# DerekRowell/AudioSDR

Hardware: AMD Instinct MI355X
Metric: Msamples/s through full SSB demod chain, batched 128-sample blocks (higher is better)
Workload: dtype f32

## Files before the change

### audiosdr_amd/csrc/asdr_kernels.hip

```cpp
#include <hip/hip_runtime.h>
#include <stdint.h>
#include <stddef.h>
#include <string.h>
#include <stdlib.h>
#include <type_traits>

#include "asdr_device.h"
#include "asdr_tables.h"
#include "../../include/asdr.h"

#ifndef ASDR_STRIDE
#define ASDR_STRIDE 388
#endif
#ifndef ASDR_ALS_STRIDE
#define ASDR_ALS_STRIDE 392
#endif
#ifndef ASDR_PRE_STRIDE
#define ASDR_PRE_STRIDE 260
#endif
#ifndef ASDR_MW
#define ASDR_MW 1
#endif
#ifndef ASDR_MW_MIN_WAVES
#define ASDR_MW_MIN_WAVES 64
#endif
#ifndef ASDR_MW_SHARE
#define ASDR_MW_SHARE 7
#endif
#ifndef ASDR_MW_PRIO
#define ASDR_MW_PRIO 2
#endif
#ifndef ASDR_MW_FIR_RING
#define ASDR_MW_FIR_RING 1
#endif
#ifndef ASDR_C16
#define ASDR_C16 0
#endif
#ifndef ASDR_C16_MIN_WAVES
#define ASDR_C16_MIN_WAVES 64
#endif
#ifndef ASDR_STATE_POLICY
#define ASDR_STATE_POLICY 1
#endif
#ifndef ASDR_NT_LOADS
#define ASDR_NT_LOADS 2
#endif
#ifndef ASDR_PIPE_PK_MASK
#define ASDR_PIPE_PK_MASK 8
#endif
#ifndef ASDR_PIPE_CHUNK
#define ASDR_PIPE_CHUNK 8
#endif
#ifndef ASDR_WAVES_PER_EU
#define ASDR_WAVES_PER_EU 3
#endif
#ifndef ASDR_ALS_WAVES_PER_EU
#define ASDR_ALS_WAVES_PER_EU 3
#endif
#ifndef ASDR_ALS_K_WAVES_PER_EU
#define ASDR_ALS_K_WAVES_PER_EU 3
#endif
#ifndef ASDR_POST_BOUNDS
#define ASDR_POST_BOUNDS ASDR_WAVES_PER_EU
#endif
#ifndef ASDR_PLL_LANES
#define ASDR_PLL_LANES 64
#endif
#ifndef ASDR_ABLATE
#define ASDR_ABLATE 0
#endif
#ifndef ASDR_STREAM_R1_CARRY
#define ASDR_STREAM_R1_CARRY 0
#endif
#ifndef ASDR_PIPE_BANK_SELECT
#define ASDR_PIPE_BANK_SELECT 0
#endif

#define W0 0
#define W1 128
#define PH 256
#define XP 0
#define ASDR_COMPACT_ROWS(stride) ((stride) < 500)
#define SCR0 387
#define NB_B 2
#define NB_MSKB 0
#define NB_CB 68
#define AGC_GV 128
#define AGC_TAB 256
#define ALS_OUT W0

#define PI_D 3.1415926535897932384626433832795

typedef float v4f __attribute__((ext_vector_type(4)));

#define ABL_NB 1
#define ABL_IF 2
#define ABL_SAM 4
#define ABL_MIX 8
#define ABL_HIL 16
#define ABL_ENV 32
#define ABL_AF 64
#define ABL_AGC 128
#define ABL_ALS 256
#define ABL_ON(x) (!(ASDR_ABLATE & (x)))

__constant__ float c_bq_pool[ASDR_N_BQ_TABLES][ASDR_BQ_COEFS];
__constant__ float c_hilbert[ASDR_HILBERT_TAPS];
__constant__ float c_sine[ASDR_SINE_TABLE_LEN];
__constant__ float c_mask_val[8];

extern "C" int asdr_kernels_upload_tables(void) {
  if (hipMemcpyToSymbol(HIP_SYMBOL(c_bq_pool), asdr_bq_pool, sizeof(asdr_bq_pool)) != hipSuccess) return -1;
  if (hipMemcpyToSymbol(HIP_SYMBOL(c_hilbert), asdr_hilbert_taps, sizeof(asdr_hilbert_taps)) != hipSuccess) return -1;
  if (hipMemcpyToSymbol(HIP_SYMBOL(c_sine), asdr_sine_table, sizeof(asdr_sine_table)) != hipSuccess) return -1;
  {
    const float val[8] = {0.0f, 1.0f, (float)0.933, (float)0.750, (float)0.500, (float)0.250, (float)0.067, 1.0f};
    if (hipMemcpyToSymbol(HIP_SYMBOL(c_mask_val), val, sizeof val) != hipSuccess) return -1;
  }
  return 0;
}

#ifdef ASDR_FENCE
#define SCHED_FENCE() __builtin_amdgcn_sched_barrier(0)
#else
#define SCHED_FENCE() do { } while (0)
#endif
#include "asdr_fir.h"
__device__ __forceinline__ double div_by_const(double x, double c, double r) {
  const double q0 = x * r;
  const double rem = __builtin_fma(-q0, c, x);
  return __builtin_fma(rem, r, q0);
// ... 136 lines not shown
  auto step = [&](auto edge_tag, const int c) {
    constexpr bool EDGE = decltype(edge_tag)::value;
    const int cn = c - st;
    float x[C], p[C], y[C];
#if ASDR_PIPE_BANK_SELECT
#pragma unroll
    for (int j = 0; j < C; ++j) x[j] = __int_as_float(__builtin_amdgcn_update_dpp(__float_as_int(xn[j]), __float_as_int(yo[j]), 0x114, 0xF, 0xE, false));
#elif ASDR_PIPE_CHUNK != 8
#pragma unroll
    for (int j = 0; j < C; ++j) { const float d = dpp_row_shr1(yo[j]); x[j] = s0 ? xn[j] : d; }
#else
    asm("s_mov_b64 vcc, %[m]\n\ts_nop 1\n\t"
        "v_cndmask_b32_dpp %[x0], %[y0], %[n0], vcc row_shr:1 row_mask:0xf bank_mask:0xf bound_ctrl:1\n\t"
        "v_cndmask_b32_dpp %[x1], %[y1], %[n1], vcc row_shr:1 row_mask:0xf bank_mask:0xf bound_ctrl:1\n\t"
        "v_cndmask_b32_dpp %[x2], %[y2], %[n2], vcc row_shr:1 row_mask:0xf bank_mask:0xf bound_ctrl:1\n\t"
        "v_cndmask_b32_dpp %[x3], %[y3], %[n3], vcc row_shr:1 row_mask:0xf bank_mask:0xf bound_ctrl:1\n\t"
        "v_cndmask_b32_dpp %[x4], %[y4], %[n4], vcc row_shr:1 row_mask:0xf bank_mask:0xf bound_ctrl:1\n\t"
        "v_cndmask_b32_dpp %[x5], %[y5], %[n5], vcc row_shr:1 row_mask:0xf bank_mask:0xf bound_ctrl:1\n\t"
        "v_cndmask_b32_dpp %[x6], %[y6], %[n6], vcc row_shr:1 row_mask:0xf bank_mask:0xf bound_ctrl:1\n\t"
        "v_cndmask_b32_dpp %[x7], %[y7], %[n7], vcc row_shr:1 row_mask:0xf bank_mask:0xf bound_ctrl:1"
        : [x0] "=&v"(x[0]), [x1] "=&v"(x[1]), [x2] "=&v"(x[2]), [x3] "=&v"(x[3]), [x4] "=&v"(x[4]), [x5] "=&v"(x[5]), [x6] "=&v"(x[6]), [x7] "=&v"(x[7])
        : [y0] "v"(yo[0]), [y1] "v"(yo[1]), [y2] "v"(yo[2]), [y3] "v"(yo[3]), [y4] "v"(yo[4]), [y5] "v"(yo[5]), [y6] "v"(yo[6]), [y7] "v"(yo[7]),
          [n0] "v"(xn[0]), [n1] "v"(xn[1]), [n2] "v"(xn[2]), [n3] "v"(xn[3]), [n4] "v"(xn[4]), [n5] "v"(xn[5]), [n6] "v"(xn[6]), [n7] "v"(xn[7]),
          [m] "s"(s0m)
        : "vcc");
#endif
    {
      const int nc = (c + 1 < ASDR_N / C) ? c + 1 : ASDR_N / C - 1;
#pragma unroll
      for (int q = 0; q < C / 4; ++q) { const float4 t = reinterpret_cast<const float4 *>(row)[nc * (C / 4) + q]; xn[4 * q] = t.x; xn[4 * q + 1] = t.y; xn[4 * q + 2] = t.z; xn[4 * q + 3] = t.w; }
    }
#if ASDR_PIPE_CHUNK == 8
    if constexpr (PK) {
    {
      const v2f B0 = (v2f){b0, b0}, B1 = (v2f){b1, b1}, B2 = (v2f){b2, b2};
      v2f P[6];
      P[0] = (v2f){x2, x[2]}; P[1] = (v2f){x1, x[3]};
#pragma unroll
      for (int k = 0; k < 4; ++k) P[2 + k] = (v2f){x[k], x[k + 4]};
#pragma unroll
      for (int k = 0; k < 4; ++k) {
        v2f t = B0 * P[2 + k]; t += B1 * P[1 + k]; t += B2 * P[k];
        p[k] = t.x; p[k + 4] = t.y;
      }
    }
    } else
#endif
    {
#pragma unroll
    for (int j = 0; j < C; ++j) {
      const float xm1 = (j >= 1) ? x[j - 1] : x1, xm2 = (j >= 2) ? x[j - 2] : ((j == 1) ? x1 : x2);
      float t = b0 * x[j]; t += b1 * xm1; t += b2 * xm2;
      p[j] = t;
    }
    }
#pragma unroll
    for (int j = 0; j < C; ++j) {
      const float ym1 = (j >= 1) ? y[j - 1] : y1, ym2 = (j >= 2) ? y[j - 2] : ((j == 1) ? y1 : y2);
      float t = p[j] + a1 * ym1; t += a2 * ym2;
      y[j] = t;
    }
    const bool act = !EDGE || ((cn >= 0) && (cn < ASDR_N / C));
    if (act) { x1 = x[C - 1]; x2 = x[C - 2]; y1 = y[C - 1]; y2 = y[C - 2]; }
#pragma unroll
    for (int j = 0; j < C; ++j) yo[j] = y[j];
    if (on && act && st == 3) {
#pragma unroll
      for (int q = 0; q < C / 4; ++q) reinterpret_cast<float4 *>(row)[cn * (C / 4) + q] = make_float4(y[4 * q], y[4 * q + 1], y[4 * q + 2], y[4 * q + 3]);
    }
  };
#if ASDR_PIPE_CHUNK != 8
#pragma unroll 1
  for (int c = 0; c < NSTEP; ++c) step(std::true_type{}, c);
#else
#pragma unroll 1
  for (int c = 0; c < 3; ++c) step(std::true_type{}, c);
#pragma unroll 1
  for (int c = 3; c < 15; c += 2) { step(std::false_type{}, c); step(std::false_type{}, c + 1); }
  step(std::false_type{}, 15);
#pragma unroll 1
  for (int c = 16; c < NSTEP; ++c) step(std::true_type{}, c);
#endif
  sv[0] = x1; sv[1] = x2; sv[2] = y1; sv[3] = y2;
}

__device__ __forceinline__ void load16(const float *p, float *v) {
  const float4 *q = reinterpret_cast<const float4 *>(p);
#pragma unroll
  for (int r = 0; r < 4; ++r) { float4 t = q[r]; v[4 * r] = t.x; v[4 * r + 1] = t.y; v[4 * r + 2] = t.z; v[4 * r + 3] = t.w; }
}
__device__ __forceinline__ void load8(const float *p, float *v) {
  const float4 *q = reinterpret_cast<const float4 *>(p);
  const float4 a = q[0], b = q[1];
  v[0] = a.x; v[1] = a.y; v[2] = a.z; v[3] = a.w; v[4] = b.x; v[5] = b.y; v[6] = b.z; v[7] = b.w;
}
__device__ __forceinline__ void load4(const float *p, float *v) {
  const float4 a = *reinterpret_cast<const float4 *>(p);
  v[0] = a.x; v[1] = a.y; v[2] = a.z; v[3] = a.w;
}
__device__ __forceinline__ void store4(float *p, const float *v) { *reinterpret_cast<float4 *>(p) = make_float4(v[0], v[1], v[2], v[3]); }
__device__ __forceinline__ void store4_nt(float *p, const float *v) {
  typedef float f4v __attribute__((ext_vector_type(4)));
  const f4v tv = {v[0], v[1], v[2], v[3]};
  __builtin_nontemporal_store(tv, reinterpret_cast<f4v *>(p));
}
__device__ __forceinline__ int4 load_int4_nt(const int4 *p) {
  typedef int i4v __attribute__((ext_vector_type(4)));
  const i4v t = __builtin_nontemporal_load(reinterpret_cast<const i4v *>(p));
  return make_int4(t[0], t[1], t[2], t[3]);
}
__device__ __forceinline__ void load4_nt(const float *p, float *v) {
  typedef float f4v __attribute__((ext_vector_type(4)));
  const f4v t = __builtin_nontemporal_load(reinterpret_cast<const f4v *>(p));
  v[0] = t[0]; v[1] = t[1]; v[2] = t[2]; v[3] = t[3];
}
__device__ __forceinline__ void store_int4_nt(int4 *p, int4 v) {
  typedef int i4v __attribute__((ext_vector_type(4)));
  const i4v tv = {v.x, v.y, v.z, v.w};
  __builtin_nontemporal_store(tv, reinterpret_cast<i4v *>(p));
}
template <bool PLAIN> __device__ __forceinline__ void store4_state(float *p, const float *v) { if constexpr (PLAIN) store4(p, v); else store4_nt(p, v); }
template <bool PLAIN> __device__ __forceinline__ void store_int4_state(int4 *p, int4 v) { if constexpr (PLAIN) *p = v; else store_int4_nt(p, v); }
__device__ __forceinline__ void store4e(float *p, const float *v) { *reinterpret_cast<float4 *>(p) = make_float4(v[0], v[2], v[4], v[6]); }
__device__ __forceinline__ void store8(float *p, const float *v) {
  float4 *q = reinterpret_cast<float4 *>(p);
  q[0] = make_float4(v[0], v[1], v[2], v[3]); q[1] = make_float4(v[4], v[5], v[6], v[7]);
}

__device__ __forceinline__ double div_i16_by_32767(double x) {
  return __builtin_fma(x, 0x1.0002000400080p-15, x * 0x1.0002000400080p-75);
}
__device__ __forceinline__ void scale8(const int16_t *s, double g, float *out, bool unit = false) {
  if (unit) {
#pragma unroll
    for (int j = 0; j < 8; ++j) { const float x = (float)s[j]; out[j] = __builtin_fmaf(x, 0x1.0002p-15f, x * 0x1.0002p-45f); }
    return;
  }
#pragma unroll
  for (int j = 0; j < 8; ++j) {
    out[j] = (float)(div_i16_by_32767((double)s[j]) * g);
    if ((j & 1) == 1) SCHED_FENCE();
  }
}
#define ASDR_MASK_MAGIC 0x14c4005000006ull
__device__ __forceinline__ float mask_decode_byte(float tabv, uint32_t group4, uint32_t word, int k) {
  const uint32_t sh = (k == 0) ? (word << 2) : (word >> (8 * k - 2));
  const uint32_t addr = (sh & 0x1Cu) | group4;
  return __int_as_float(__builtin_amdgcn_ds_bpermute((int)addr, __float_as_int(tabv)));
}
__device__ __forceinline__ uint32_t mask_encode(float v) {
  const uint32_t idx = (__float_as_uint(v) >> 21) & 0x1Fu;
  return (uint32_t)(ASDR_MASK_MAGIC >> ((idx * 3u - 36u) & 63u)) & 7u;
}
__device__ __forceinline__ uint32_t mask_encode4(float4 mv) {
  const uint32_t c0 = mask_encode(mv.x), c1 = mask_encode(mv.y), c2 = mask_encode(mv.z), c3 = mask_encode(mv.w);
  return c0 | (c1 << 8) | (c2 << 16) | (c3 << 24);
}

#define ALS_TAP(q, wh) ((((q) & 1) ? (wh) : 0) + ((q) >> 1))
template <bool CHECKED, int WH>
__device__ __forceinline__ float als_dot(const float *w, const float *x, int top, int M) {
  float y = 0.0f;
  int q = 0;
#pragma unroll 2
  for (; q + 4 <= M; q += 4) {
    const float2 we = *reinterpret_cast<const float2 *>(w + (q >> 1)), wo = *reinterpret_cast<const float2 *>(w + WH + (q >> 1));
// ... 337 lines not shown
        for (int j = 0; j < 4; ++j) XI[j] = L[XB + i0 + 4 * j];
        epoch(std::false_type{}, std::integral_constant<int, 0>{}, ep0, E, F, XI);
        epoch(std::false_type{}, std::integral_constant<int, 1>{}, ep0 + 1, E, F, XI);
        epoch(std::false_type{}, std::integral_constant<int, 2>{}, ep0 + 2, E, F, XI);
        epoch(std::false_type{}, std::integral_constant<int, 3>{}, ep0 + 3, E, F, XI);
      }
#pragma unroll
      for (int g = 0; g < 7; ++g) L[AW + WH * h + 4 * g + tq] = wr[g];
      WAVE_SYNC();
    } else
    if (__any(als_en && adaptive)) {
#pragma unroll 1
      for (int ep = -1; ep < 32; ++ep) {
        const int base = (ep < 0) ? 0 : 4 * ep + 1;
        const int cntn = (ep < 0) ? 1 : ((ep == 31) ? 3 : 4);
        const int n = base + (s8 & 3);
        const bool mine = als_en && adaptive && (s8 < cntn);
        if (als_safe) {
          const int i = 128 + n, h = s8 >> 2;
          float y = 0.0f;
          if (als_m_default) y = als_dot_split_const<ALS_M_DEFAULT>(L + AW + WH * h, L + XB + (i - D - h), h);
          else if (als_m_uniform) y = als_dot_split_uniform(L + AW + WH * h, L + XB + (i - D - h), M_u, h);
          else if (als_en && adaptive) y = als_dot_split(L + AW + WH * h, L + XB + (i - D - h), M, h);
          if (mine) {
            const float e = L[XB + i] - y;
            L[OUT + n] = notch ? e : y;
            if ((n & 3) == 0) L[SCR] = e;
          }
        } else if (mine) {
          if constexpr (!COMPACT) {
            const int i = 128 + n;
            const float y = als_dot<true, WH>(L + AW, L + XB, i - D, M);
            const float e = L[XB + i] - y;
            L[OUT + n] = notch ? e : y;
            if ((n & 3) == 0) L[SCR] = e;
          }
        }
        WAVE_SYNC();
        const int nu = (ep < 0) ? 0 : 4 * ep + 4;
        if (als_en && adaptive && nu < ASDR_N) {
          const float e = L[SCR];
          const int iu = 128 + nu;
          if (als_m_default) {
            als_tap_update_const<ALS_M_DEFAULT>(L + XB + iu - D - s8, L + AW + ALS_TAP(s8, WH), e, lam, s8);
          } else if (als_m_uniform && als_safe) {
            const float *xq = L + XB + iu - D - s8;
            float *wq = L + AW + ALS_TAP(s8, WH);
            const int nk = (M_u - s8 + 7) >> 3, nk_max = (M_u + 7) >> 3;
#pragma unroll 1
            for (int k0 = 0; k0 < nk_max; k0 += 8) {
              float xv[8], wv[8];
#pragma unroll
              for (int j = 0; j < 8; ++j) { xv[j] = xq[-8 * (k0 + j)]; wv[j] = wq[4 * (k0 + j)]; }
#pragma unroll
              for (int j = 0; j < 8; ++j) { const float gq = e * xv[j]; const float dq = lam * gq; const float wn = wv[j] + dq; wv[j] = (k0 + j < nk) ? wn : wv[j]; }
#pragma unroll
              for (int j = 0; j < 8; ++j) wq[4 * (k0 + j)] = wv[j];
            }
          } else if (als_safe) {
#pragma unroll 2
            for (int q = s8; q < M; q += 8) { const float gq = e * L[XB + iu - D - q]; const float dq = lam * gq; L[AW + ALS_TAP(q, WH)] += dq; }
          } else {
            if constexpr (!COMPACT) {
              for (int q = s8; q < M; q += 8) { const float gq = e * (((iu - D - q) >= 0 && (iu - D - q) < 256) ? L[XB + (iu - D - q)] : 0.0f); const float dq = lam * gq; L[AW + ALS_TAP(q, WH)] += dq; }
            }
          }
        }
        WAVE_SYNC();
      }
    }
}
template <int STRIDE, bool HAS_ALS, bool HAS_SAM, bool UNIFORM, int WAVES, int ROLE = 0, bool ONEBLK_ = false, int FIR_HELPERS = 1, bool UPAR = false>
__device__ __forceinline__ void asdr_update_body(const UpdateArgs &a, float *lds_wg) {
  constexpr bool C16 = (STRIDE == 320);
  constexpr bool PRE_ROLE = (ROLE == 4 || ROLE == 8), POST_ROLE = (ROLE == 5 || ROLE == 9 || ROLE == 10), LOOPED_ROLE = (ROLE == 7 || ROLE == 8 || ROLE == 9 || ROLE == 10);
  constexpr bool DO1 = (ROLE == 0 || ROLE == 1 || PRE_ROLE || ROLE == 6 || ROLE == 7), DO2 = (ROLE == 0 || ROLE == 2 || POST_ROLE || ROLE == 6 || ROLE == 7),
                 DO3 = (ROLE == 0 || ROLE == 3 || POST_ROLE || ROLE == 6 || ROLE == 7);
  constexpr bool TO_ALS = (ROLE == 6 || ROLE == 7 || ROLE == 10);
  constexpr bool ONEBLK = ONEBLK_ || (ROLE >= 4 && !LOOPED_ROLE);
  constexpr bool ALS_FULL_OPT = ASDR_COMPACT_ROWS(STRIDE) && ONEBLK;
  constexpr bool STREAM = (ROLE >= 1 && ROLE <= 3);
  constexpr bool PIPE_PK = ((ASDR_PIPE_PK_MASK & 1) && HAS_ALS) || ((ASDR_PIPE_PK_MASK & 2) && !HAS_ALS && !HAS_SAM && ROLE == 0) ||
                           ((ASDR_PIPE_PK_MASK & 4) && (HAS_SAM || ROLE > 3)) || ((ASDR_PIPE_PK_MASK & 8) && STREAM);
  if (ROLE == 0 && a.run_if != nullptr && *a.run_if == 0u) return;
  constexpr bool MW = (WAVES > 1) && !HAS_SAM && (ROLE == 0);
  constexpr int MW_SHARE = MW ? ASDR_MW_SHARE : 0;
  const int wave = (WAVES > 1) ? (int)(threadIdx.x >> 6) : 0;
  constexpr bool ORDERED = (ROLE == 0) && !HAS_ALS && !HAS_SAM && UNIFORM && ONEBLK_ && (STRIDE == ASDR_STRIDE);
  constexpr bool ST_PLAIN = ORDERED && (ASDR_STATE_POLICY >= 1), LD_PLAIN = ORDERED && (ASDR_STATE_POLICY >= 2);
  const int wg_l = (ORDERED && a.wg_reverse != 0u) ? (int)(gridDim.x - 1u - blockIdx.x) : (int)blockIdx.x;
  const int mw_rel = MW ? (int)(((uint32_t)wave - blockIdx.x) & (uint32_t)(WAVES - 1)) : 0;
  float *const mwx = lds_wg + WAVES * 8 * STRIDE;
  int *const mw_flags = reinterpret_cast<int *>(lds_wg + WAVES * 8 * STRIDE + 8 * WAVES * 16 + 260) + 4;
  constexpr int MWX = 16;
  auto mw_channel = [&](int q) -> int { const int sidx = wg_l * (8 * WAVES) + q; return (sidx < a.n_sched) ? a.direct_ch0 + sidx : a.n_channels; };
  const int wave_g = STREAM ? wg_l % a.stream_waves : wg_l * WAVES + wave;
  float *const lds = lds_wg + wave * 8 * STRIDE;
  const int lane = threadIdx.x & 63, c8 = lane >> 3, s8_ = lane & 7;
  float *const sine = HAS_SAM ? lds_wg + WAVES * 8 * STRIDE : nullptr;
  if (HAS_SAM) for (int i = lane; i < ASDR_SINE_TABLE_LEN; i += 64) sine[i] = c_sine[i];

  int4 slot = make_int4(a.n_channels, 0, 0, 0);
  const bool mw_pad = MW && (wave_g * 8 >= a.n_sched);
  if (UNIFORM && a.direct_ch0 >= 0) slot = make_int4(mw_pad ? a.n_channels : a.direct_ch0 + wave_g * 8 + c8, (int)a.direct_mode, (int)a.direct_flags, (int)((a.direct_lo & 0xFFu) | (wave_g == 0 ? a.lo_writer_bit : 0u)));
  else if (WAVES == 1 || wave_g * 8 < a.n_sched) slot = *reinterpret_cast<const int4 *>(a.sched + wave_g * 8 + c8);
  else { const ChanParams *pd = a.params + a.n_channels; slot.y = (int)pd->mode; slot.z = (int)pd->flags; }
  const int ch_ = slot.x;
  const bool valid = (UNIFORM && !mw_pad) || (ch_ < a.n_channels);
  const int loff_ = c8 * STRIDE;
#define P (*Pp)
  const ChainConsts K = a.k;
  auto pv = [](float x) -> float { if constexpr (UPAR) asm volatile("" : "+v"(x)); return x; };

  const uint32_t mode = UNIFORM ? (uint32_t)__builtin_amdgcn_readfirstlane(slot.y) : (uint32_t)slot.y;
  const uint32_t pflags = UNIFORM ? (uint32_t)__builtin_amdgcn_readfirstlane(slot.z) : (uint32_t)slot.z;
  const uint32_t lo_slot = UNIFORM ? (uint32_t)__builtin_amdgcn_readfirstlane(slot.w) : 0u;
  const bool is_ssb = DO2 && ((mode == ASDR_USBmode) || (mode == ASDR_LSBmode) || (mode == ASDR_CW_USBmode) ||
                              (mode == ASDR_CW_LSBmode) || (mode == ASDR_WSPRmode));
  const bool is_am = !C16 && (mode == ASDR_AMmode), is_sam = (HAS_SAM || ROLE >= 4) && (mode == ASDR_SAMmode);
  const bool sub_q = (mode == ASDR_USBmode) || (mode == ASDR_CW_USBmode) || (mode == ASDR_WSPRmode);
  const bool nb_en = DO1 && (pflags & ASDR_F_NB_EN), af_en = DO3 && (pflags & ASDR_F_AF_EN), agc_en = DO3 && (pflags & ASDR_F_AGC_EN);
  const bool als_en = HAS_ALS && (pflags & ASDR_F_ALS_EN);
  const bool muted = pflags & ASDR_F_MUTED;
  const float two_pi = K.two_pi_f;
  WAVE_SYNC();
  uint32_t seen_in = 0u, seen_free = 0u, seen_lo = 0u, sig_pending = 0u;
  float carry_phase = 0.0f, carry_fsh = 0.0f;
  uint32_t carry_hs = 0u;
  int4 pf_in[4] = {make_int4(0, 0, 0, 0), make_int4(0, 0, 0, 0), make_int4(0, 0, 0, 0), make_int4(0, 0, 0, 0)};
  constexpr bool R2_ONE_TRIP = (ROLE == 2) && (FIR_HELPERS == 3);
  v4f r2n_key = (v4f){0.f, 0.f, 0.f, 0.f}, r2n_c4[4], r2n_s4[4], r2n_vi[4], r2n_vq[4];
  bool r2_pref = false;
  uint32_t r2_look_in = 0u, r2_look_lo = 0u;
  float4 r1_if_s4 = make_float4(0.f, 0.f, 0.f, 0.f);
  float r1_if_cf[5] = {0.f, 0.f, 0.f, 0.f, 0.f}, r1_gain_i = 0.f, r1_gain_q = 0.f;
  uint32_t *const my_prog = STREAM ? a.stream_prog + (ROLE - 1) * a.stream_waves + wave_g : nullptr;

  constexpr bool UNIT_OK = (ONEBLK && ROLE == 0) || ROLE == 1;
  static_assert(!C16 || (ONEBLK && UNIFORM && !HAS_ALS && !HAS_SAM && WAVES == 1 && ROLE == 0), "the 16-waves-per-CU form is the plain uniform one-block kernel");
#pragma unroll 1
  for (int blk = 0; blk < (ONEBLK ? 1 : a.n_blocks); ++blk) {
    int s8 = s8_; asm volatile("" : "+v"(s8));
    int loff = loff_; asm volatile("" : "+v"(loff));
    int ch = ch_; asm volatile("" : "+v"(ch));
    int lane_i = lane; asm volatile("" : "+v"(lane_i));
#ifdef ASDR_TIMELINE
    if (STREAM && a.taps != nullptr && wave_g == 0 && lane == 0) (reinterpret_cast<unsigned long long *>(a.taps) + 64 * (3 + ROLE) + 32 * (blk & 1))[16] = clock64();
#endif
    if (STREAM) {
      uint32_t *prog = a.stream_prog, *err = a.stream_err;
      const uint32_t b1 = (uint32_t)blk + 1u, freed = (blk >= ASDR_STREAM_DEPTH) ? (uint32_t)(blk - ASDR_STREAM_DEPTH + 1) : 0u;
      const bool need_in = (ROLE != 1) && seen_in < b1, need_free = (ROLE != 3) && seen_free < freed;
      if ((need_in || need_free) && sig_pending) { stream_signal(my_prog, sig_pending, lane); sig_pending = 0u; }
      if (need_in) { seen_in = stream_wait(prog + (ROLE - 2) * a.stream_waves + wave_g, b1, err, a.stream_spin_limit); if (seen_in == ASDR_STREAM_FAIL) break; }
      if (need_free) { seen_free = stream_wait(prog + ROLE * a.stream_waves + wave_g, freed, err, a.stream_spin_limit); if (seen_free == ASDR_STREAM_FAIL) break; }
    }
    const ChanParams *Pp = UPAR ? &a.uni : row_ptr(a.params, (uint32_t)ch * (uint32_t)sizeof(ChanParams));
    ChanSmall *S = row_ptr(a.small, (uint32_t)ch * (uint32_t)sizeof(ChanSmall));
    float *L = lds + loff;
    int *Li = reinterpret_cast<int *>(L);
    constexpr bool PLB = (ASDR_PIPE_BANK_SELECT != 0);
#define pl_st (PLB ? ((lane_i & 15) >> 2) : (s8 & 3))
#define pl_iq (PLB ? (lane_i & 1) : (s8 >> 2))
#define pl_c (PLB ? (2 * (lane_i >> 4) + ((lane_i >> 1) & 1)) : (lane_i >> 3))
#define pa_c (PLB ? (2 * (lane_i >> 4) + (lane_i & 1)) : (lane_i >> 3))
#define pa_real (PLB ? ((lane_i & 3) < 2) : ((lane_i & 7) < 4))
// ... 1062 lines not shown
        }
        S->am_carrier = lvl; carrier_now = lvl; carrier_fresh = true;
        if (ROLE == 2) {
          float *xc = a.xch_c + (size_t)ch * ASDR_STREAM_DEPTH + (size_t)(blk % ASDR_STREAM_DEPTH);
          asm volatile("global_store_dword %0, %1, off sc1\n\ts_nop 0" :: "v"(xc), "v"(lvl) : "memory");
        }
      }
    }
    if (is_sam && pll_locked) {
#pragma unroll 1
      for (int h = 0; h < 2; ++h) {
        float vi[8], vq[8];
        load8(L + W0 + kA + 64 * h, vi); load8(L + W1 + kA + 64 * h, vq);
        TAP8(ASDR_TAP_MIX_I, h, vi); TAP8(ASDR_TAP_MIX_Q, h, vq);
        store8(L + W0 + kA + 64 * h, vq);
      }
    }
    if ((ROLE == 0 || ROLE == 6 || ROLE == 7) && !is_ssb && !is_am && mode != ASDR_SAMmode) {
      float z[16];
      DEFINE_ALL_PATHS(z, 16);
      if (a.audio_prev != nullptr) {
        const float *ap = row_ptr(a.audio_prev, (uint32_t)ch * 512u + 4u * (uint32_t)kF);
#pragma unroll
        for (int m = 0; m < 4; ++m) load4(ap + 32 * m, z + 4 * m);
      }
#pragma unroll
      for (int m = 0; m < 4; ++m) store4(L + W0 + kF + 32 * m, z + 4 * m);
    }
    WAVE_SYNC();
    TL(10);
    TAP_ROW(ASDR_TAP_DEMOD, W0);
    if (ROLE == 2 || ROLE == 3) {
      float *xb = a.xch_b + ((size_t)ch * ASDR_STREAM_DEPTH + (size_t)(blk % ASDR_STREAM_DEPTH)) * ASDR_N + kF;
      if (ROLE == 2) {
        v4f v[4];
#pragma unroll
        for (int m = 0; m < 4; ++m) v[m] = *reinterpret_cast<const v4f *>(L + W0 + kF + 32 * m);
        xch_store4x4(xb, v[0], v[1], v[2], v[3]);
        sig_pending = (uint32_t)blk + 1u;
        continue;
      } else {
        v4f v[4];
        if (is_am) {
          const float *xc = a.xch_c + (size_t)ch * ASDR_STREAM_DEPTH + (size_t)(blk % ASDR_STREAM_DEPTH);
          asm volatile("global_load_dword %4, %6, off sc1\n\t"
                       "global_load_dwordx4 %0, %5, off sc1\n\tglobal_load_dwordx4 %1, %5, off offset:128 sc1\n\t"
                       "global_load_dwordx4 %2, %5, off offset:256 sc1\n\tglobal_load_dwordx4 %3, %5, off offset:384 sc1\n\t"
                       "s_waitcnt vmcnt(0)"
                       : "=&v"(v[0]), "=&v"(v[1]), "=&v"(v[2]), "=&v"(v[3]), "=&v"(carrier_now) : "v"(xb), "v"(xc) : "memory");
          carrier_fresh = true;
        } else
        xch_load4x4(xb, v[0], v[1], v[2], v[3]);
        if (sig_pending) { if (lane == 0) __hip_atomic_store(my_prog, sig_pending, __ATOMIC_RELAXED, __HIP_MEMORY_SCOPE_AGENT); sig_pending = 0u; }
#pragma unroll
        for (int m = 0; m < 4; ++m) *reinterpret_cast<v4f *>(L + W0 + kF + 32 * m) = v[m];
        WAVE_SYNC();
      }
    }

    float4 agc_t4[5];
#pragma unroll
    for (int r = 0; r < 5; ++r) agc_t4[r] = make_float4(0.f, 0.f, 0.f, 0.f);
    float agc_al_a = 0.f, agc_be_a = 0.f, agc_al_r = 0.f, agc_be_r = 0.f, agc_sg = 0.f;
    uint32_t agc_hang = 0u;
    if (ABL_ON(ABL_AGC) && agc_en) {
      agc_al_a = P.agc_alpha_att; agc_be_a = P.agc_beta_att; agc_al_r = P.agc_alpha_rel; agc_be_r = P.agc_beta_rel;
      agc_sg = P.agc_static_gain; agc_hang = P.agc_hang_count;
      const float *gtab = a.agc_tab + (size_t)agc_tab_idx * ASDR_AGC_TAB_ROW;
      if constexpr (!C16) {
#pragma unroll
      for (int r = 0; r < 5; ++r) { const int q = s8 + 8 * r; if (q < 33) agc_t4[r] = reinterpret_cast<const float4 *>(gtab)[q]; }
      }
    }
    if constexpr ((MW_SHARE & 1) != 0) {
      if (ABL_ON(ABL_AF) && af_en) {
        TL(21);
        __syncthreads();
        TL(22);
        if (mw_audio_duty) {
          if (ASDR_MW_PRIO) __builtin_amdgcn_s_setprio(ASDR_MW_PRIO);
          const int st = pl_st;
          float sv[4];
          sv[0] = af_s4.x; sv[1] = af_s4.y; sv[2] = af_s4.z; sv[3] = af_s4.w;
          biquad_pipe<PIPE_PK>(lds_wg + (16 * (mw_rel - 1) + mw_casc) * STRIDE + W0, true, st, af_cf, sv);
          *reinterpret_cast<float4 *>(&mw_af_S->af_state[4 * st]) = make_float4(sv[0], sv[1], sv[2], sv[3]);
          if (ASDR_MW_PRIO) __builtin_amdgcn_s_setprio(0);
        }
        TL(23);
        __syncthreads();
        TL(24);
      }
    } else
    if (ABL_ON(ABL_AF) && __any(af_en)) {
      const int st = pl_st;
      const bool on = af_en_pa && pa_real;
      float sv[4];
      sv[0] = af_s4.x; sv[1] = af_s4.y; sv[2] = af_s4.z; sv[3] = af_s4.w;
      ChanSmall *const Saf = Spa;
      biquad_pipe<PIPE_PK>(Lpa + W0, on, st, af_cf, sv);
      if (on) *reinterpret_cast<float4 *>(&Saf->af_state[4 * st]) = make_float4(sv[0], sv[1], sv[2], sv[3]);
      WAVE_SYNC();
    }
    TL(11);
    TAP_ROW(ASDR_TAP_AUDIO_FILT, W0);

    if (ABL_ON(ABL_AGC) && __any(agc_en)) {
      const float *tab = C16 ? a.agc_tab + (size_t)agc_tab_idx * ASDR_AGC_TAB_ROW : L + AGC_TAB;
      const float gain_in = agc_gain_in;
      float av16[16];
      DEFINE_ALL_PATHS(av16, 16);
      float blockmax = 0.0f;
      if (agc_en) {
#pragma unroll
        for (int h = 0; h < 2; ++h) {
          float au[8];
          load8(L + W0 + kA + 64 * h, au);
#pragma unroll
          for (int j = 0; j < 8; ++j) { const float ax = fabsf(au[j]); av16[8 * h + j] = (ax > 1.0f) ? 1.0f : ax; }
          float mx = av16[8 * h];
#pragma unroll
          for (int u = 1; u < 8; ++u) mx = fmaxf(mx, av16[8 * h + u]);
          blockmax = (h == 0) ? mx : fmaxf(blockmax, mx);
        }
        blockmax = fmaxf(blockmax, __int_as_float(__builtin_amdgcn_update_dpp(0, __float_as_int(blockmax), 0xB1, 0xF, 0xF, true)));
        blockmax = fmaxf(blockmax, __int_as_float(__builtin_amdgcn_update_dpp(0, __float_as_int(blockmax), 0x4E, 0xF, 0xF, true)));
        blockmax = fmaxf(blockmax, __int_as_float(__builtin_amdgcn_update_dpp(0, __float_as_int(blockmax), 0x141, 0xF, 0xF, true)));
      }
      const float am_level = (float)(2.0 * (double)(carrier_fresh ? carrier_now : agc_carrier0));
      const float am_clamped = (am_level > 1.0f) ? 1.0f : am_level;
      const bool agc_quiet = __all(!(agc_en && lead) || (agc_hc0 >= 128u && agc_hang >= 8u && !((is_am ? am_clamped : blockmax) > agc_old0)));
      if (agc_en && !agc_quiet) {
        if constexpr (!C16) {
#pragma unroll
        for (int r = 0; r < 5; ++r) { const int q = s8 + 8 * r; if (q < 33) *reinterpret_cast<float4 *>(L + AGC_TAB + 4 * q) = agc_t4[r]; }
        }
        store8(L + AGC_GV + kA, av16); store8(L + AGC_GV + kA + 64, av16 + 8);
      }
      if (!agc_quiet) WAVE_SYNC();
      TL(12);
      if (agc_quiet) {
        if (agc_en && lead) {
          S->agc_hang_counter = agc_hc0 - 128u;
          status = (status & ~ASDR_S_AGC_ACTIVE) | (((double)gain_in < 0.99) ? ASDR_S_AGC_ACTIVE : 0u);
        }
      }
      {
      float agc_old_end = 0.0f; uint32_t agc_hc_end = 0u;
      auto agc_chain = [&](auto own_tag, float *Lc, ChanSmall *Sc, float old0, uint32_t hc0, float g_in, float al_a, float be_a, float al_r, float be_r, uint32_t hang,
                           bool am, float am_lvl) -> float {
        float old_abs = old0;
        uint32_t hc = hc0;
        float gv = -1.0f;
        if (am) {
#pragma unroll 1
          for (int i = 0; i < ASDR_N; i += 4) *reinterpret_cast<float4 *>(Lc + AGC_GV + i) = make_float4(am_lvl, am_lvl, am_lvl, am_lvl);
        }
        float x_[8];
        load8(Lc + AGC_GV, x_);
#pragma unroll 1
        for (int i2 = 0; i2 < ASDR_N; i2 += 16) {
          float xn_[8];
#pragma unroll
        for (int half = 0; half < 2; ++half) {
          const int i = i2 + 8 * half;
          float *x = half ? xn_ : x_, *xn = half ? x_ : xn_;
          float gvv[8];
          load8(Lc + AGC_GV + ((i + 8 < ASDR_N) ? i + 8 : i), xn);
          float mx = x[0];
#pragma unroll
          for (int u = 1; u < 8; ++u) mx = fmaxf(mx, x[u]);
          const bool no_release = __all(hc >= 8u && hang >= 8u);
          if (no_release && __all(!(mx > old_abs))) {
            hc -= 8u;
#pragma unroll
            for (int u = 0; u < 8; ++u) gvv[u] = gv;
          } else if (no_release) {
            uint32_t hcb = hc;
#pragma unroll
            for (int u = 0; u < 8; ++u) {
              const float av = x[u];
              const bool att = av > old_abs;
              if (MW || __any(att)) {
// ... 925 lines not shown
```

Before: 87790.

## Add one-sample-skew biquad cascade pipeline with inline-asm DPP handover for audio filter

Adds a new biquad cascade implementation in which each of four stage lanes is skewed by one sample and receives its input from the previous stage through a DPP row_shr:1 cndmask, written as hand-scheduled inline assembly over 8-sample chunks. It is enabled by default for the non-ALS, non-SAM role-0 path via a new mask macro and replaces the previous biquad_pipe there. The intent is to shorten the per-sample dependency chain and drop the per-step edge masking of the old skewed pipeline. In exchange it adds fragile inline asm that clobbers vcc, hand-managed write offsets, and a static_assert that rules out combining it with the packed or bank-select variants.

```diff
diff --git a/audiosdr_amd/csrc/asdr_kernels.hip b/audiosdr_amd/csrc/asdr_kernels.hip
--- a/audiosdr_amd/csrc/asdr_kernels.hip
+++ b/audiosdr_amd/csrc/asdr_kernels.hip
@@ -47,6 +47,9 @@
 #endif
 #ifndef ASDR_PIPE_PK_MASK
 #define ASDR_PIPE_PK_MASK 8
+#endif
+#ifndef ASDR_PIPE_SKEW1_MASK
+#define ASDR_PIPE_SKEW1_MASK 2
 #endif
 #ifndef ASDR_PIPE_CHUNK
 #define ASDR_PIPE_CHUNK 8
@@ -349,6 +352,94 @@
   for (int c = 16; c < NSTEP; ++c) step(std::true_type{}, c);
 #endif
   sv[0] = x1; sv[1] = x2; sv[2] = y1; sv[3] = y2;
+}
+
+__device__ __forceinline__ void load8(const float *p, float *v);
+#define ASDR_BQ_SLOT(YJ, NJ, XA, XB, YA, YB) \
+  "v_mul_f32 %[" YJ "], %[b1], %[" XA "]\n\t" \
+  "v_mul_f32 %[t1], %[b2], %[" XB "]\n\t" \
+  "v_mul_f32 %[t2], %[a1], %[" YA "]\n\t" \
+  "v_mul_f32 %[t3], %[a2], %[" YB "]\n\t" \
+  "v_cndmask_b32_dpp %[" XB "], %[" YA "], %[" NJ "], vcc row_shr:1 row_mask:0xf bank_mask:0xf bound_ctrl:1\n\t" \
+  "v_mul_f32 %[t0], %[b0], %[" XB "]\n\t" \
+  "v_add_f32 %[t0], %[t0], %[" YJ "]\n\t" \
+  "v_add_f32 %[t0], %[t0], %[t1]\n\t" \
+  "v_add_f32 %[t0], %[t0], %[t2]\n\t" \
+  "v_add_f32 %[" YJ "], %[t0], %[t3]\n\t"
+__device__ __forceinline__ void biquad_pipe_skew1(float *row, bool on, int st, const float *cf, float *sv) {
+  const float b0 = cf[0], b1 = cf[1], b2 = cf[2], a1 = cf[3], a2 = cf[4];
+  float x1 = sv[0], x2 = sv[1], y1 = sv[2], y2 = sv[3];
+  float xn[8], yp[8];
+  load8(row, xn);
+  const bool s0 = (st == 0), wr = on && (st == 3);
+  const unsigned long long s0m = __ballot(s0);
+  auto slot = [&](auto edge_tag, const int t, const float xin) -> float {
+    constexpr bool EDGE = decltype(edge_tag)::value;
+    const float d = dpp_row_shr1(y1);
+    const float x = s0 ? xin : d;
+    float acc = b0 * x; acc += b1 * x1; acc += b2 * x2; acc += a1 * y1; acc += a2 * y2;
+    if constexpr (EDGE) {
+      const int n = t - st;
+      const bool act = (n >= 0 && n < ASDR_N);
+      asm volatile("" : "+v"(acc));
+      x2 = act ? x1 : x2; x1 = act ? x : x1; y2 = act ? y1 : y2; y1 = act ? acc : y1;
+    } else { x2 = x1; x1 = x; y2 = y1; y1 = acc; }
+    return acc;
+  };
+  {
+    float nx[8];
+    load8(row + 8, nx);
+#pragma unroll
+    for (int j = 0; j < 3; ++j) yp[j] = slot(std::true_type{}, j, xn[j]);
+#pragma unroll
+    for (int j = 3; j < 8; ++j) yp[j] = slot(std::false_type{}, j, xn[j]);
+#pragma unroll
+    for (int j = 0; j < 8; ++j) xn[j] = nx[j];
+  }
+  auto step = [&](auto pf_tag, const int c) {
+    constexpr bool PF = decltype(pf_tag)::value;
+    float nx[8], y[8], t0, t1, t2, t3;
+    if constexpr (PF) load8(row + 8 * (c + 1), nx);
+    asm("s_mov_b64 vcc, %[m]\n\t"
+        ASDR_BQ_SLOT("y0", "n0", "xa", "xb", "p1", "p2")
+        ASDR_BQ_SLOT("y1", "n1", "xb", "xa", "y0", "p1")
+        ASDR_BQ_SLOT("y2", "n2", "xa", "xb", "y1", "y0")
+        ASDR_BQ_SLOT("y3", "n3", "xb", "xa", "y2", "y1")
+        ASDR_BQ_SLOT("y4", "n4", "xa", "xb", "y3", "y2")
+        ASDR_BQ_SLOT("y5", "n5", "xb", "xa", "y4", "y3")
+        ASDR_BQ_SLOT("y6", "n6", "xa", "xb", "y5", "y4")
+        ASDR_BQ_SLOT("y7", "n7", "xb", "xa", "y6", "y5")
+        : [y0] "=&v"(y[0]), [y1] "=&v"(y[1]), [y2] "=&v"(y[2]), [y3] "=&v"(y[3]), [y4] "=&v"(y[4]), [y5] "=&v"(y[5]), [y6] "=&v"(y[6]), [y7] "=&v"(y[7]),
+          [t0] "=&v"(t0), [t1] "=&v"(t1), [t2] "=&v"(t2), [t3] "=&v"(t3), [xa] "+v"(x1), [xb] "+v"(x2)
+        : [n0] "v"(xn[0]), [n1] "v"(xn[1]), [n2] "v"(xn[2]), [n3] "v"(xn[3]), [n4] "v"(xn[4]), [n5] "v"(xn[5]), [n6] "v"(xn[6]), [n7] "v"(xn[7]),
+          [b0] "v"(b0), [b1] "v"(b1), [b2] "v"(b2), [a1] "v"(a1), [a2] "v"(a2), [p1] "v"(y1), [p2] "v"(y2), [m] "s"(s0m)
+        : "vcc");
+    y1 = y[7]; y2 = y[6];
+    if (wr) {
+      float4 *const o = reinterpret_cast<float4 *>(row + 8 * (c - 1));
+      o[0] = make_float4(yp[3], yp[4], yp[5], yp[6]); o[1] = make_float4(yp[7], y[0], y[1], y[2]);
+    }
+#pragma unroll
+    for (int j = 0; j < 8; ++j) { yp[j] = y[j]; if constexpr (PF) xn[j] = nx[j]; }
+  };
+#pragma unroll 1
+  for (int c = 1; c < 15; c += 2) { step(std::true_type{}, c); step(std::true_type{}, c + 1); }
+  step(std::false_type{}, 15);
+  {
+    float y[3];
+#pragma unroll
+    for (int j = 0; j < 3; ++j) y[j] = slot(std::true_type{}, ASDR_N + j, 0.0f);
+    if (wr) {
+      float4 *const o = reinterpret_cast<float4 *>(row + ASDR_N - 8);
+      o[0] = make_float4(yp[3], yp[4], yp[5], yp[6]); o[1] = make_float4(yp[7], y[0], y[1], y[2]);
+    }
+  }
+  sv[0] = x1; sv[1] = x2; sv[2] = y1; sv[3] = y2;
+}
+#undef ASDR_BQ_SLOT
+template <bool PK, bool SKEW1>
+__device__ __forceinline__ void biquad_run(float *row, bool on, int st, const float *cf, float *sv) {
+  if constexpr (SKEW1) biquad_pipe_skew1(row, on, st, cf, sv); else biquad_pipe<PK>(row, on, st, cf, sv);
 }
 
 __device__ __forceinline__ void load16(const float *p, float *v) {
@@ -852,6 +943,9 @@
   constexpr bool STREAM = (ROLE >= 1 && ROLE <= 3);
   constexpr bool PIPE_PK = ((ASDR_PIPE_PK_MASK & 1) && HAS_ALS) || ((ASDR_PIPE_PK_MASK & 2) && !HAS_ALS && !HAS_SAM && ROLE == 0) ||
                            ((ASDR_PIPE_PK_MASK & 4) && (HAS_SAM || ROLE > 3)) || ((ASDR_PIPE_PK_MASK & 8) && STREAM);
+  constexpr bool PIPE_SKEW1 = !STREAM && !C16 && (((ASDR_PIPE_SKEW1_MASK & 1) && HAS_ALS) || ((ASDR_PIPE_SKEW1_MASK & 2) && !HAS_ALS && !HAS_SAM && ROLE == 0) ||
+                                          ((ASDR_PIPE_SKEW1_MASK & 4) && (HAS_SAM || ROLE > 3)));
+  static_assert(!(PIPE_SKEW1 && (PIPE_PK || ASDR_PIPE_BANK_SELECT)), "the one-sample skew has no packed form and hands over by row_shr:1");
   if (ROLE == 0 && a.run_if != nullptr && *a.run_if == 0u) return;
   constexpr bool MW = (WAVES > 1) && !HAS_SAM && (ROLE == 0);
   constexpr int MW_SHARE = MW ? ASDR_MW_SHARE : 0;
@@ -2080,7 +2174,7 @@
           const int st = pl_st;
           float sv[4];
           sv[0] = af_s4.x; sv[1] = af_s4.y; sv[2] = af_s4.z; sv[3] = af_s4.w;
-          biquad_pipe<PIPE_PK>(lds_wg + (16 * (mw_rel - 1) + mw_casc) * STRIDE + W0, true, st, af_cf, sv);
+          biquad_run<PIPE_PK, PIPE_SKEW1>(lds_wg + (16 * (mw_rel - 1) + mw_casc) * STRIDE + W0, true, st, af_cf, sv);
           *reinterpret_cast<float4 *>(&mw_af_S->af_state[4 * st]) = make_float4(sv[0], sv[1], sv[2], sv[3]);
           if (ASDR_MW_PRIO) __builtin_amdgcn_s_setprio(0);
         }
@@ -2095,7 +2189,7 @@
       float sv[4];
       sv[0] = af_s4.x; sv[1] = af_s4.y; sv[2] = af_s4.z; sv[3] = af_s4.w;
       ChanSmall *const Saf = Spa;
-      biquad_pipe<PIPE_PK>(Lpa + W0, on, st, af_cf, sv);
+      biquad_run<PIPE_PK, PIPE_SKEW1>(Lpa + W0, on, st, af_cf, sv);
       if (on) *reinterpret_cast<float4 *>(&Saf->af_state[4 * st]) = make_float4(sv[0], sv[1], sv[2], sv[3]);
       WAVE_SYNC();
     }
```

Measured after the change: 89950 (median of 6 runs). +2.5%, better.
